# nomadkaraoke/python-audio-separator

Measured on AMD Instinct MI355X. Metric: audio-sec separated / wall-sec (RTF), UVR-MDX-NET 44.1kHz stereo, 1/2/4/8 GPU, higher is better.
Workload: dtype f32 (I/O and accumulators; matrix products on the 16-bit pipe from block-scaled two-part fp16 operands, 22-bit products -- see arithmetic; fp32-exact setting timed in arithmetic_ab)

## Files before the change

### python-audio-separator_amd/csrc/asx.hip

```cpp
#include <hip/hip_runtime.h>

#include <algorithm>
#include <atomic>
#include <cmath>
#include <cstdarg>
#include <cstdio>
#include <cstdlib>
#include <cstring>
#include <functional>
#include <map>
#include <string>
#include <mutex>
#include <vector>

#include "../../include/asx.h"
#include "knobs.h"
#include "resample_plan.h"
#include "flac_dec_plan.h"

static void grant_lds(const void *kernel, int bytes) {
  static std::mutex mu;
  static std::map<const void *, int> granted;
  std::lock_guard<std::mutex> lock(mu);
  int &g = granted[kernel];
// ... 43 lines not shown
  int (*norm)(int32_t);
  const char *refusal = nullptr;
  int shipped = 0;
} kOptions[] = {
    {"winograd", &asx_engine::winograd, &EngineKnobs::winograd, opt_nonneg,
     "asx_set_option: winograd = %d names a superseded kernel generation that only an experimental build carries "
     "(python build.py --experimental); this library has 0 (direct kernel) and 3 (the default)", 3},
    {"winograd_stationary", &asx_engine::winos, &EngineKnobs::winos, opt_nonneg,
     "asx_set_option: the weight-stationary Winograd kernel (measured slower) is in experimental builds only (python build.py --experimental)"},
    {"winograd_bf16x6", &asx_engine::wino6, &EngineKnobs::wino6, opt_nonneg},
    {"gemm_bf16x6", &asx_engine::gemm_bf16x6, &EngineKnobs::gemm_bf16x6, opt_onoff},
    {"gemm_f16x3", &asx_engine::gemm_f16x3, &EngineKnobs::gemm_f16x3, opt_onoff},
    {"conv_direct_f16x3", &asx_engine::conv3h, &EngineKnobs::conv3h, opt_nonneg},
    {"conv_fuse_input", &asx_engine::conv_fuse_input, &EngineKnobs::conv_fuse_input, opt_onoff},
    {"conv3h_partial_scratch", &asx_engine::conv3h_ps, &EngineKnobs::conv3h_ps, opt_onoff},
    {"conv_down_bf16x6", &asx_engine::down6, &EngineKnobs::down6, opt_onoff},
    {"conv_up_bf16x6", &asx_engine::up6, &EngineKnobs::up6, opt_onoff},
    {"gemm_pair_images", &asx_engine::pair_images, &EngineKnobs::pair_images, opt_onoff,
     "asx_set_option: gemm_pair_images = 1 needs an experimental build (python build.py --experimental): the pair-image reader measured no "
     "faster in the nets and is not in the default library"},
};

static const EngineOption *find_option(const char *fn, const char *key) {
  for (const EngineOption &o : kOptions)
    if (!strcmp(key, o.key)) return &o;
  set_err("%s: unknown option '%s'", fn, key);
  return nullptr;
}

extern "C" {
// ... 186 lines not shown
  e->d_tw3.release();
  e->d_hann3.release();
  e->seam3.release();
  e->d_zeros.release();
  free_conv(e->first);
  free_conv(e->final_);
  for (auto &b : e->enc) free_block(b);
  for (auto &b : e->dec) free_block(b);
  free_block(e->mid);
  for (auto &c : e->ds) free_conv(c);
  for (auto &c : e->us) free_conv(c);
  e->spec_in.release();
  e->spec_out.release();
  for (auto &r : e->R) r.release();
  e->c3h_ps.release();
  e->H.release();
  e->frames.release();
  e->chunk_out.release();
  e->d_starts.release();
  e->d_nact.release();
  e->d_peak.release();
  e->d_demixed.release();
  e->d_div.release();
  for (DevBuf *b : {&e->pool_wave, &e->pool_nsong, &e->pool_songs, &e->pool_div, &e->pool_peak}) b->release();
  for (auto &sk : e->skip) sk.release();
  if (e->v3) v3_destroy(e->v3);
  if (e->rof) rof_destroy(e->rof);
  hd_drop_clones(e);
  if (e->ht) ht_destroy(e->ht);
  if (e->hd) hd_destroy(e->hd);
// ... 251 lines not shown
  hipStream_t s = reinterpret_cast<hipStream_t>(stream);
  HIPCHK(hipSetDevice(e->device));
  asx_plan p;
  CHK(asx_plan_query(e, N, flags, &p));
  REQUIRE(k0 >= 0 && k1 <= p.n_chunks && k0 <= k1, "chunk range [%d,%d) outside [0,%d)", k0, k1, p.n_chunks);
  const bool match = (flags & ASX_FLAG_MATCH_MIX) != 0;
  const bool need_net = !match;
  if (need_net && !e->net_ready) {
    set_err("asx_demix: net weights not committed");
    return ASX_ERR_STATE;
  }
  const int nk = k1 - k0;
  if (nk == 0) return ASX_OK;
  const int per = even_batches(nk, pick_batch(e));
  CHK(ensure_workspace(e, per, need_net));
  const bool win = windowed_mode(e, flags);
  CHK(e->d_starts.ensure((size_t)nk * 8));
  CHK(e->d_nact.ensure((size_t)nk * 8));
  hipLaunchKernelGGL(chunk_table_kernel, dim3((unsigned)((nk + 255) / 256)), dim3(256), 0, s, k0, nk, p.step, p.chunk_size,
                     p.padded_len, win ? 1 : 0, reinterpret_cast<int64_t *>(e->d_starts.p), reinterpret_cast<int64_t *>(e->d_nact.p));
  HIPCHK(hipGetLastError());
  const int T = e->cfg.segment_size;
  const int64_t C = p.chunk_size;
  const size_t spec_elems = (size_t)4 * T * e->cfg.dim_f;
  for (int b0 = 0; b0 < nk; b0 += per) {
    const int B = std::min(per, nk - b0);
    const int64_t *ds = reinterpret_cast<const int64_t *>(e->d_starts.p) + b0;
    const int64_t *dn = reinterpret_cast<const int64_t *>(e->d_nact.p) + b0;
    CHK(stft_launch(e, mix_dev, ds, N, B, C, T, e->spec_in.f(), 1, 3, 1.0f, s));
    const float *spec_final = e->spec_in.f();
// ... 87 lines not shown
  }
  const int nk = (int)total;
  const asx_plan &p0 = plans[0];
  const int64_t C = p0.chunk_size;
  const int T = e->cfg.segment_size;
  const bool win = windowed_mode(e, flags);
  const double *hann = (e->fft3 && e->d_hann3.p) ? reinterpret_cast<const double *>(e->d_hann3.p) : nullptr;
  const int maxB = pick_batch(e);
  const int nbatch = (nk + maxB - 1) / maxB;
  const int per = (nk + nbatch - 1) / nbatch;
  std::map<int64_t, int64_t> div_off;
  int64_t div_floats = 0;
  for (int i = 0; i < n; ++i)
    if (div_off.emplace(Ns[i], div_floats).second) div_floats += (Ns[i] + 3) / 4 * 4;
  CHK(ensure_workspace(e, per, need_net));
  CHK(e->d_starts.ensure((size_t)nk * 8));
  CHK(e->d_nact.ensure((size_t)nk * 8));
  CHK(e->pool_wave.ensure((size_t)nk * 8));
  CHK(e->pool_nsong.ensure((size_t)nk * 8));
  CHK(e->pool_songs.ensure((size_t)n * sizeof(PoolSong)));
  CHK(e->pool_div.ensure((size_t)div_floats * 4));
  CHK(e->chunk_out.ensure((size_t)nk * 2 * C * 4));
  if (e->fft3) CHK(e->seam3.ensure((size_t)per * 2 * std::max(1, T / knobs().fft3_g) * 2 * 5 * f3::HOP * 4));
  float *chunks = e->chunk_out.f();
  const bool geom4 = knobs().finalize4 && C % 4 == 0 && p0.step % 4 == 0 && p0.trim % 4 == 0;
  int64_t blk = 0;
  for (int g0 = 0; g0 < n; g0 += POOL_GROUP) {
    PoolGroup g{};
    g.n_songs = std::min(POOL_GROUP, n - g0);
    g.song0 = g0;
// ... 641 lines not shown
  } else {
    set_err("asx_op_conv: unknown op '%s'", op);
    return ASX_ERR_INVALID;
  }
  ConvLayer L;
  DevBuf dx, dy, dskip;
  BufGuard g{{&dx, &dy, &dskip, &L.w, &L.b, &L.wu, &L.wu2, &L.wu3, &L.wus, &L.wu6, &L.wu6h, &L.w3h, &L.wd6, &L.wup6}};
  CHK(conv_setup(L, kind, cin, cout, relu ? 1 : 0));
  CHK(conv_pack(L, w_host, b_host, e->winograd));
  CHK(to_dev(dx, x_host, (size_t)B * cin * t * f));
  const size_t ny = (size_t)B * cout * to * fo;
  CHK(dy.ensure(ny * 4));
  HIPCHK(hipMemset(dy.p, 0xff, ny * 4));
  if (kind == CK_UP) CHK(to_dev(dskip, aux_host, ny));
  CHK(e->c3h_ps.ensure(conv3h_ps_need(L, B, t, f)));
  CHK(conv_launch(e, L, dx.f(), dskip.f(), dy.f(), B, t, f, nullptr));
  CHK(to_host(y_host, dy, ny));
  return ASX_OK;
}

int asx_op_tdf(asx_engine *e, const float *x_host, int32_t B, int32_t c, int32_t t, int32_t k, const float *w_host,
               const float *bias_host, int32_t n, const float *scale_host, const float *shift_host,
               const float *res_host, float *y_host) {
  REQUIRE(e && x_host && w_host && scale_host && shift_host && y_host && B > 0 && c > 0 && t > 0 && k > 0 && n > 0,
          "asx_op_tdf: bad argument");
  HIPCHK(hipSetDevice(e->device));
  TdfLayer L;
  DevBuf dx, dy, dres;
  BufGuard g{{&dx, &dy, &dres, &L.w, &L.bias, &L.scale, &L.shift}};
  CHK(tdf_pack(L, n, k, c, w_host, bias_host, scale_host, shift_host));
// ... 572 lines not shown
    if (br.rof)
      hipLaunchKernelGGL(roformer_finalize_pool_kernel, dim3((unsigned)blocks, br.rows * 2), dim3(256), 0, s, table, n, br.S, C, pp.step,
                         e->rof->d_window.f());
    else
      hipLaunchKernelGGL(mdxc_finalize_pool_kernel, dim3((unsigned)blocks, br.rows * 2), dim3(256), 0, s, table, n, br.S, C, pp.step, pp.front,
                         (float)pp.overlap);
  });
}

static int mdxc_pool_demix(asx_engine *e, const char *fn, bool rof, const asx_mdxc_song *songs, const MdxcPoolPlan &pp, void *stream) {
  hipStream_t s = reinterpret_cast<hipStream_t>(stream);
  HIPCHK(hipSetDevice(e->device));
  const MdxcBranch br = mdxc_branch(e, rof);
  const int nk = pp.total(), per = mdxc_pool_per_pass(nk, e->cfg.max_batch);
  CHK(rof ? rof_ensure_workspace(e, per) : v3_ensure_workspace(e, per));
  CHK(br.chunk_out.ensure((size_t)nk * br.chunk_floats(pp) * 4));
  int64_t blk = 0;
  CHK(mdxc_pool_tables(e, fn, br, songs, pp, br.chunk_out.f(), s, &blk));
  CHK(mdxc_pool_chunks(e, br, pp, 0, nk, br.chunk_out.f(), s));
  return mdxc_pool_fold(e, br, songs, pp, blk, s);
}

static int mdxc_pool_plan(const char *fn, asx_engine *e, bool rof, const asx_mdxc_song *songs, int32_t n_songs, int64_t geom, MdxcPoolPlan &pp) {
  REQUIRE(e && n_songs >= 0 && (songs || n_songs == 0), "%s: null argument", fn);
  std::vector<int64_t> Ns((size_t)n_songs);
  for (int i = 0; i < n_songs; ++i) {
    REQUIRE(songs[i].mix_dev && songs[i].out_dev, "%s: null pointer in song %d", fn, i);
    REQUIRE(songs[i].n_samples >= 1, "%s: song %d: n_samples must be >= 1", fn, i);
    Ns[i] = songs[i].n_samples;
  }
// ... 746 lines not shown
```

### python-audio-separator_amd/csrc/engine_core.h

```cpp
#pragma once

static thread_local char g_err[512] = "";
static void set_err(const char *fmt, ...) {
  va_list ap;
  va_start(ap, fmt);
  vsnprintf(g_err, sizeof(g_err), fmt, ap);
  va_end(ap);
}
#define HIPCHK(x)                                                                       \
  do {                                                                                  \
    hipError_t e_ = (x);                                                                \
    if (e_ != hipSuccess) {                                                             \
      set_err("%s:%d %s -> %s", __FILE__, __LINE__, #x, hipGetErrorString(e_));         \
      return ASX_ERR_HIP;                                                               \
    }                                                                                   \
  } while (0)
#define CHK(x)                    \
  do {                            \
    int r_ = (x);                 \
    if (r_ != ASX_OK) return r_;  \
  } while (0)
#define REQUIRE(cond, ...)        \
  do {                            \
    if (!(cond)) {                \
// ... 92 lines not shown
struct Block {
  std::vector<ConvLayer> tfc;
  TdfLayer tdf0, tdf1;
  int c = 0, t = 0, f = 0;
};

struct ProfRec {
  int cls;
  int nprod;
  hipEvent_t a, b;
  double flops, bytes;
};

struct RsTable {
  ResamplePlan plan;
  DevBuf tab;
};

struct V3Net;
struct RofNet;
struct HtNet;
struct HdNet;
struct VrNet;
struct EnsCtx;

struct W3Entry {
  const float *w;
  int N, K, cin;
  int kind;
  void *img;
// ... 30 lines not shown
  DevBuf d_tw3, seam3;
  bool fft3 = false;
  bool fft3p = false;
  DevBuf d_zeros;
  bool net_begun = false, net_ready = false;
  asx_net_config net{};
  std::map<std::string, std::vector<float>> host_tensors;
  ConvLayer first, final_;
  std::vector<Block> enc, dec;
  Block mid;
  std::vector<ConvLayer> ds, us;
  int ws_batch = 0;
  DevBuf spec_in, spec_out, R[3], H, HE, frames, chunk_out, d_starts, d_nact, d_peak, d_demixed;
  DevBuf pool_wave, pool_nsong, pool_songs, pool_div, pool_peak;
  DevBuf c3h_ps;
  DevBuf gn_part;
  DevBuf d_div;
  DivKey div_key;
  DevBuf sinc_tab;
  DevBuf flac_cycles;
  long long flac_block_cycles = 0, flac_crc16_cycles = 0;
  DevBuf flac_frames, flac_off;
  DevBuf flacdec_list, flacdec_slots, flacdec_accept;
  std::vector<flacdec::Accept> flacdec_accept_host;
  int64_t flacdec_n_samples = -1, flacdec_n_frames = 0;
  int32_t flacdec_channels = 0, flacdec_bps = 0, flacdec_max_bs = 0;
  size_t flacdec_slot_off = 0;
  std::vector<RsTable *> rs_tabs;
  std::mutex rs_mu;
  hipEvent_t div_ev = nullptr;
  hipStream_t div_stream = nullptr;
  std::vector<DevBuf> skip;
  int winograd = 3;
  int winos = 0;
  int gemm_bf16x6 = 1;
  int gemm_f16x3 = 1;
  int wino6 = 144;
  int conv3h = 144;
  int conv3h_ps = 1;
  int conv_fuse_input = 1;
  int down6 = 1;
  int up6 = 1;
  int pair_images = 0;
  std::vector<W3Entry> w3;
  std::mutex w3_mu;
  bool prof = false;
  int prof_nprod = 0;
  std::vector<ProfRec> recs;
};

static int pick_batch(const asx_engine *e) { return e->cfg.max_batch > 0 ? e->cfg.max_batch : 64; }

#include "batching.h"

// ... 74 lines not shown
```

### python-audio-separator_amd/csrc/engine_mdx.h

```cpp
#pragma once

template <class CFG>
static void launch_conv_t(const ConvArgs &a, int nblk, hipStream_t s) {
  grant_lds(&conv_mfma_kernel<CFG>, CFG::LDS_BYTES);
  hipLaunchKernelGGL(conv_mfma_kernel<CFG>, dim3(nblk), dim3(256), CFG::LDS_BYTES, s, a);
}

static int conv_tile_h(int kind) { return kind == CK_UP ? 4 : 8; }

static int pick_nrep_conv(int cout) {
  const int ct = (cout + 15) / 16;
  int best = 1, best_pad = 1 << 30;
  for (int n = 3; n >= 1; --n) {
    const int pad = ((ct + n - 1) / n) * n - ct;
    if (pad < best_pad) {
      best_pad = pad;
      best = n;
    }
  }
  return best;
}
static int pick_nrep_up(int cout) {
  const int ct = (cout + 15) / 16;
  if (knobs().up_nrep == 4 && (4 * ct) % 4 == 0) return 4;
// ... 207 lines not shown

static bool conv3h_takes(const asx_engine *e, const ConvLayer &L, bool dma, const float *res, int act, int T, int F, int64_t y_bstride, const float *y) {
#ifdef ASX_EXPERIMENTAL_KERNELS
  if (e->winos == 1 && L.wus.p != nullptr) return false;
#endif
  return L.kind == CK_3X3 && e->winograd == 3 && e->gemm_bf16x6 > 0 && e->gemm_f16x3 > 0 && e->conv3h > 0 && L.cin <= e->conv3h && L.w3h.p != nullptr && dma &&
         res == nullptr && (act == ACT_RELU || act == ACT_NONE) && F % 32 == 0 && (int64_t)Conv3hCfg::C * T * F < ((int64_t)1 << 29) &&
         y_bstride % 4 == 0 && (reinterpret_cast<uintptr_t>(y) & 15) == 0;
}

static size_t conv3h_ps_need(const ConvLayer &L, int B, int T, int F) {
  if (L.kind != CK_3X3 || L.w3h.p == nullptr || L.cin <= Conv3hCfg::C || F % 32 != 0 || B <= 0 || T <= 0) return 0;
  return (size_t)Conv3hCfg::ps_bytes(B, (T + 3) / 4, F / 32);
}

static int conv_launch(asx_engine *e, const ConvLayer &L, const float *x, const float *skip, float *y, int B, int T,
                       int F, hipStream_t s, const ConvView &v = ConvView()) {
  ConvArgs a{};
  a.x = x;
  a.wp = L.w.f();
  a.bias = L.b.f();
  a.skip = skip;
  a.res = v.res;
  a.zeros = e->d_zeros.f();
  a.y = y;
  a.B = B;
  a.Cin = L.cin;
  a.Cout = L.cout;
  a.T = T;
  a.F = F;
// ... 70 lines not shown
        case 1: return k12 ? gos(&conv_winos_kernel<12, 1>, WinoSCfg<12>::LDS_BYTES) : gos(&conv_winos_kernel<24, 1>, WinoSCfg<24>::LDS_BYTES);
        case 2: return k12 ? gos(&conv_winos_kernel<12, 2>, WinoSCfg<12>::LDS_BYTES) : gos(&conv_winos_kernel<24, 2>, WinoSCfg<24>::LDS_BYTES);
        case 4: return k12 ? gos(&conv_winos_kernel<12, 4>, WinoSCfg<12>::LDS_BYTES) : gos(&conv_winos_kernel<24, 4>, WinoSCfg<24>::LDS_BYTES);
        case 5: return k12 ? gos(&conv_winos_kernel<12, 5>, WinoSCfg<12>::LDS_BYTES) : gos(&conv_winos_kernel<24, 5>, WinoSCfg<24>::LDS_BYTES);
        case 13: return k12 ? gos(&conv_winos_kernel<12, 13>, WinoSCfg<12>::LDS_BYTES) : gos(&conv_winos_kernel<24, 13>, WinoSCfg<24>::LDS_BYTES);
        default: break;
      }
    }
    if (ragged) return k12 ? gos(&conv_winos_kernel<12, 0, true>, WinoSCfg<12>::LDS_BYTES) : gos(&conv_winos_kernel<24, 0, true>, WinoSCfg<24>::LDS_BYTES);
    return k12 ? gos(&conv_winos_kernel<12, 0, false>, WinoSCfg<12>::LDS_BYTES) : gos(&conv_winos_kernel<24, 0, false>, WinoSCfg<24>::LDS_BYTES);
  }
#endif
  if (conv3h_takes(e, L, dma, v.res, a.act, T, F, a.y_bstride, y)) {
    const int nb = L.cin / Conv3hCfg::C;
    const int tilesT = (T + 3) / 4, tilesF = F / 32;
    int bw = 32;
    double best = 1e30;
    for (int cand : {32, 16, 8}) {
      if ((tilesT * cand) % 32 != 0) continue;
      const int tps = tilesT * cand / 32;
      const int bands = (tilesF + cand - 1) / cand, items = B * bands;
      const double cost = (double)(bands * cand) / tilesF * (tps + 1.0) / tps * (double)((items + 7) / 8) / (items / 8.0);
      if (cost < best - 1e-9) {
        best = cost;
        bw = cand;
      }
    }
    if (best > 1e29) bw = 32;
    grant_lds(&conv3h_kernel<0, false>, Conv3hCfg::LDS_BYTES);
    grant_lds(&conv3h_kernel<0, true>, Conv3hCfg::LDS_BYTES);
    grant_lds(&conv3h_kernel<0, false, true>, Conv3hCfg::LDS_BYTES);
    grant_lds(&conv3h_kernel<0, false, false, 1>, Conv3hCfg::LDS_BYTES);
    grant_lds(&conv3h_kernel<0, false, false, 2>, Conv3hCfg::LDS_BYTES);
    grant_lds(&conv3h_kernel<0, false, false, 3>, Conv3hCfg::LDS_BYTES);
    const int64_t plane = (int64_t)T * F;
    const bool ps = e->conv3h_ps > 0 && nb > 1;
    const int64_t ps_item = Conv3hCfg::ps_item_bytes(tilesT, tilesF);
    REQUIRE(!ps || (ps_item < ((int64_t)1 << 32) && e->c3h_ps.p != nullptr && e->c3h_ps.bytes >= conv3h_ps_need(L, B, T, F)),
            "conv3h_kernel: the partial-sum scratch is not sized for %d x %d x %d (the workspace set-up sizes it)", B, T, F);
    Conv3hArgs walk{};
    walk.B = B;
    walk.T = T;
    walk.F = F;
    walk.x_bstride = a.x_bstride;
    walk.y_bstride = a.y_bstride;
    walk.tilesT = tilesT;
    walk.tilesF = tilesF;
    walk.bw = bw;
    walk.tps = (tilesT * bw) % 32 == 0 ? tilesT * bw / 32 : tilesT;
    walk.ps = ps ? e->c3h_ps.p : nullptr;
    walk.ps_bstride = ps_item;
    return timed(e, cls, flops, bytes, s, [&]() {
      e->prof_nprod = 3;
      for (int ob = 0; ob < nb; ++ob)
        for (int ib = 0; ib < nb; ++ib) {
          Conv3hArgs ca = walk;
          ca.x = x + (int64_t)ib * Conv3hCfg::C * plane;
          ca.y = y + (int64_t)ob * Conv3hCfg::C * plane;
          ca.prev = ib > 0 && !ps ? ca.y : nullptr;
          ca.wimg = reinterpret_cast<const u32x4 *>(reinterpret_cast<const uint32_t *>(L.w3h.p) + (size_t)(ob * nb + ib) * Conv3hCfg::IMG_U32);
          ca.bias = ib == 0 ? L.b.f() + ob * Conv3hCfg::C : nullptr;
          ca.act = ib == nb - 1 ? a.act : ACT_NONE;
          if (v.fin) {
            ca.xin = v.fin_x;
// ... 796 lines not shown
    for (int r = 0; r < 3; ++r)
      if (e->R[r].f() != cur) {
        out = e->R[r].f();
        break;
      }
    CHK(conv_launch(e, e->us[i], cur, gn ? nullptr : e->skip[n - 1 - i].f(), out, B, blk.t / 2, blk.f / 2, s));
    if (gn)
      CHK(gn_launch(e, out, B, e->us[i].cout, (int64_t)blk.t * blk.f, e->us[i].gn_w, e->us[i].gn_b, nullptr, e->skip[n - 1 - i].f(), out, s));
    cur = out;
    CHK(block_forward(e, blk, cur, nullptr, B, s));
  }
  CHK(conv_launch(e, e->final_, cur, nullptr, spec_out, B, T, F, s));
  return ASX_OK;
}

static int ensure_workspace(asx_engine *e, int Bchunks, bool need_net) {
  const int T = e->cfg.segment_size, Fq = e->cfg.dim_f;
  const int mult = (need_net && e->cfg.enable_denoise) ? 2 : 1;
  const size_t Bn = (size_t)Bchunks * mult;
  CHK(e->spec_in.ensure(Bn * 4 * T * Fq * 4));
  CHK(e->frames.ensure((size_t)Bchunks * 2 * T * e->cfg.n_fft * 4));
  if (need_net) {
    CHK(e->spec_out.ensure(Bn * 4 * T * Fq * 4));
    const size_t lvl0 = Bn * e->net.g * T * Fq * 4;
    for (int i = 0; i < 3; ++i) CHK(e->R[i].ensure(lvl0));
    CHK(e->H.ensure(Bn * e->net.g * T * (Fq / std::max(1, e->net.bn)) * 4 + 256));
    CHK(e->HE.ensure(Bn * e->net.g * T * (size_t)((Fq / std::max(1, e->net.bn) + 127) / 128) * 4 + 256));
    if (e->net.norm == 1) CHK(e->gn_part.ensure(Bn * (size_t)e->net.g * (e->net.num_blocks / 2 + 1) * 16));
    const int n = e->net.num_blocks / 2;
    e->skip.resize(n);
    for (int i = 0; i < n; ++i) {
      const size_t c = (size_t)e->net.g * (i + 1), t = T >> i, f = Fq >> i;
      CHK(e->skip[i].ensure(Bn * c * t * f * 4));
    }
    size_t ps = 0;
    auto ps_block = [&](const Block &blk) {
      for (const ConvLayer &L : blk.tfc) ps = std::max(ps, conv3h_ps_need(L, (int)Bn, blk.t, blk.f));
    };
    for (const Block &blk : e->enc) ps_block(blk);
    ps_block(e->mid);
    for (const Block &blk : e->dec) ps_block(blk);
    CHK(e->c3h_ps.ensure(ps));
  }
  e->ws_batch = std::max(e->ws_batch, Bchunks);
  return ASX_OK;
}
```

### python-audio-separator_amd/csrc/engine_v3.h

```cpp
#pragma once
#include "v3_norm.h"

struct V3Norm {
  DevBuf g, b;
  int c = 0;
};

struct V3Block {
  int in_c = 0, c = 0, f = 0;
  V3Norm n_tfc1, n_tdf0, n_tdf1, n_tfc2;
  ConvLayer tfc1, tfc2, shortcut;
  TdfLayer tdf0, tdf1;
};

struct V3Net {
  asx_v3_config cfg{};
  float act_alpha = 1.f;
  bool begun = false, ready = false;
  ConvLayer first, final0, final1;
  std::vector<std::vector<V3Block>> enc, dec;
  std::vector<V3Block> mid;
  std::vector<ConvLayer> ds, us;
  std::vector<V3Norm> ds_n, us_n;
  int ws_batch = 0;
// ... 160 lines not shown
    CHK(tdf_launch(e, b.tdf0, n.A.f(), nullptr, n.H.f(), M, T, s, 0));
    const int fb = b.tdf0.n;
    CHK(v3_norm_act(e, b.n_tdf1, V3View{n.H.f(), (int64_t)b.c * T * fb}, b.c, (int64_t)T * fb, B, n.HA.f(), s));
    CHK(tdf_launch(e, b.tdf1, n.HA.f(), n.X1.f(), n.X2.f(), M, T, s, 0));
    CHK(v3_norm_act(e, b.n_tfc2, V3View{n.X2.f(), (int64_t)b.c * P}, b.c, P, B, n.A.f(), s));
    ConvView vo;
    vo.res = n.S.f();
    V3View out = last ? dest : V3View{n.XB.f(), (int64_t)b.c * P};
    vo.y_bstride = out.bstride;
    CHK(conv_launch(e, b.tfc2, n.A.f(), nullptr, out.p, B, T, F, s, vo));
    x = out;
  }
  return ASX_OK;
}

static int v3_ensure_workspace(asx_engine *e, int B) {
  V3Net &n = *e->v3;
  if (B <= n.ws_batch) return ASX_OK;
  const asx_v3_config &cf = n.cfg;
  const int T = e->cfg.segment_size, k = cf.num_subbands, Fs = e->cfg.dim_f / k;
  const int dim_c = k * cf.num_channels * 2;
  const int64_t P0 = (int64_t)T * Fs;
  const int c0 = cf.num_channels_model;
  const size_t big = (size_t)B * 2 * c0 * P0 * 4;
  CHK(n.cat0.ensure((size_t)B * (dim_c + c0) * P0 * 4));
  CHK(n.firstout.ensure((size_t)B * c0 * P0 * 4));
  CHK(n.A.ensure(big));
  CHK(n.S.ensure(big / 2));
  CHK(n.X1.ensure(big / 2));
  CHK(n.X2.ensure(big / 2));
  CHK(n.XB.ensure(big / 2));
  CHK(n.CUR.ensure(big / 2));
// ... 186 lines not shown
```

### python-audio-separator_amd/csrc/kernels_conv3h.h

```cpp
#pragma once
#include <cstring>
#include <vector>

#include "kernels_gemm3.h"

namespace asx {

struct Conv3hArgs {
  const float *x;
  float *y;
  const u32x4 *wimg;
  const float *bias;
  int B, T, F;
  int64_t x_bstride, y_bstride;
  int act;
  int tilesT, tilesF;
  int bw, tps;
  const float *prev;
  long long *dbg;
  const float *xin;
  const float *w1;
  int64_t xin_bstride;
  void *ps;
  int64_t ps_bstride;
};

struct Conv3hCfg {
  static constexpr int C = 48, CG8 = C / 8;
  static constexpr int TH = 4, TW = 32, IW = TW + 2;
  static constexpr int PSTR = C * 2;
  static constexpr int ROWB = IW * PSTR;
  static constexpr int RING = 12;
  static constexpr int PART = RING * ROWB;
  static constexpr int KGY = 3 * CG8;
  static constexpr int SPK = (KGY + 3) / 4;
  static constexpr int NST = (3 * KGY + 3) / 4;
  static constexpr int WKY = (KGY / 4) * 3 * 2 * 1024 + 3 * 2 * 512;
  static constexpr int WBYTES = 3 * WKY;
  static constexpr int W_OFF = 0, X_OFF = WBYTES, TAB_OFF = X_OFF + 2 * PART;
  static constexpr int LDS_BYTES = TAB_OFF + 64;
  static constexpr size_t IMG_U32 = WBYTES / 4 + 48;
  static constexpr int EUP = 8;

  static constexpr int PS_STORE = 1024, PS_WAVE = 6 * PS_STORE, PS_TILE = 4 * PS_WAVE;
  static constexpr int64_t ps_item_bytes(int tilesT, int tilesF) { return (int64_t)tilesF * tilesT * PS_TILE; }
  static constexpr int64_t ps_bytes(int B, int tilesT, int tilesF) { return (int64_t)B * ps_item_bytes(tilesT, tilesF); }
  static constexpr unsigned ps_wave_off(int tilesT, int strip, int jt, int r) { return (unsigned)((strip * tilesT + jt) * 4 + r) * (unsigned)PS_WAVE; }
  static constexpr int64_t ps_off(int tilesT, int tilesF, int b, int strip, int jt, int r, int k, int lane) {
    return (int64_t)b * ps_item_bytes(tilesT, tilesF) + ps_wave_off(tilesT, strip, jt, r) + k * PS_STORE + lane * 16;
  }

  enum { FULL = 0, MERGED = 1, PADDED = 2 };
  struct Stage {
    int kind, ky, kyb, sg;
    int rfrom, rto;
  };
  static constexpr int NPROG = 2;
// ... 104 lines not shown
            hh[e] = conv3h_f16_rne(us);
            ll[e] = conv3h_f16_rne(us - conv3h_f16_f(hh[e]));
          }
          const size_t pstep = half ? 512 : 1024;
          const size_t fb = (size_t)ky * CFG::WKY + (half ? (size_t)(CFG::SPK - 1) * 6144 + (size_t)(n * 2) * 512 : (size_t)sg * 6144 + (size_t)(n * 2) * 1024);
          uint32_t *dh = &img[(fb + (size_t)lane * 16) / 4], *dl = &img[(fb + pstep + (size_t)lane * 16) / 4];
          for (int e = 0; e < 4; ++e) {
            dh[e] = (uint32_t)hh[2 * e] | ((uint32_t)hh[2 * e + 1] << 16);
            dl[e] = (uint32_t)ll[2 * e] | ((uint32_t)ll[2 * e + 1] << 16);
          }
        }
    }
}

struct Conv3hWalk {
  int item, j, b, strip;
};
__device__ __forceinline__ void conv3h_walk_item(const Conv3hArgs &a, int wg, Conv3hWalk &w) {
  const int nbands = (a.tilesF + a.bw - 1) / a.bw;
  w.b = w.item / nbands;
  w.strip = (w.item - w.b * nbands) * a.bw + (wg >> 3) % a.bw;
}
__device__ __forceinline__ int conv3h_row0(const Conv3hArgs &a, int wg) { return ((wg >> 3) / a.bw) * a.tps * 4; }
__device__ __forceinline__ int conv3h_nblocks(const Conv3hArgs &a, int wg) {
  const int items = a.B * ((a.tilesF + a.bw - 1) / a.bw), x = wg & 7;
  return x < items ? ((items - x + 7) >> 3) * (a.tps + 1) : 0;
}
__device__ __forceinline__ void conv3h_walk_init(const Conv3hArgs &a, int wg, Conv3hWalk &w) {
  w.item = wg & 7;
  w.j = -1;
  conv3h_walk_item(a, wg, w);
}
__device__ __forceinline__ void conv3h_walk_next(const Conv3hArgs &a, int wg, Conv3hWalk &w) {
  if (++w.j == a.tps) {
    w.j = -1;
    w.item += 8;
    conv3h_walk_item(a, wg, w);
  }
}

__device__ __forceinline__ void conv3h_split_pair(float x0, float x1, float s, unsigned &h, unsigned &l) {
  unsigned hh = 0, ll = 0;
  asm("v_fma_mixlo_f16 %0, %1, %2, 0 op_sel_hi:[0,0,0]" : "+v"(hh) : "v"(x0), "v"(s));
  asm("v_fma_mixhi_f16 %0, %1, %2, 0 op_sel_hi:[0,0,0]" : "+v"(hh) : "v"(x1), "v"(s));
  asm("v_fma_mixlo_f16 %0, %1, %2, -%3 op_sel:[0,0,0] op_sel_hi:[0,0,1]" : "+v"(ll) : "v"(x0), "v"(s), "v"(hh));
  asm("v_fma_mixhi_f16 %0, %1, %2, -%3 op_sel:[0,0,1] op_sel_hi:[0,0,1]" : "+v"(ll) : "v"(x1), "v"(s), "v"(hh));
  h = hh;
  l = ll;
}

template <int BM>
__device__ __forceinline__ float ror8m(float keep, float from) {
// ... 17 lines not shown
  extern __shared__ float lds_f[];
  char *lds = reinterpret_cast<char *>(lds_f);
  const int tid = threadIdx.x;
  const int lane = tid & 63;
  const int wave = __builtin_amdgcn_readfirstlane(tid >> 6);
  const int wg = blockIdx.x;
  float *maxtab = reinterpret_cast<float *>(lds + CFG::TAB_OFF);
  int *exps = reinterpret_cast<int *>(lds + CFG::TAB_OFF + 32);

  {
    const u32x4 *src = a.wimg;
    u32x4 *dst = reinterpret_cast<u32x4 *>(lds + CFG::W_OFF);
    for (int i = tid; i < CFG::WBYTES / 16; i += 512) dst[i] = src[i];
  }
  const int64_t TF = (int64_t)a.T * a.F;
  const int NB = conv3h_nblocks(a, wg);
  const int row0 = conv3h_row0(a, wg);
  const unsigned plane_bytes = (unsigned)(CFG::C * TF * 4);

  if (wave >= 4) {
    const int ptid = tid - 256, pw = wave - 4;
    int row, cig, q;
    if (ptid < 160) {
      q = (ptid & 1) + 2 * ((ptid >> 3) % 5);
      cig = (ptid >> 1) & 3;
      row = ptid / 40;
    } else {
      const int u = ptid - 160;
      q = (u & 1) + 2 * ((u >> 3) % 5);
      cig = 4 + ((u >> 1) & 1);
      row = ((u >> 2) & 1) + 2 * (u / 40);
    }
// ... 11 lines not shown
        const f32x4 wv = *reinterpret_cast<const f32x4 *>(a.w1 + (cig * 8 + c) * 4);
        fr.w1[c][0] = wv.x;
        fr.w1[c][1] = wv.y;
        fr.w1[c][2] = wv.z;
        fr.w1[c][3] = wv.w;
        fr.b1[c] = a.w1[CFG::C * 4 + cig * 8 + c];
      }
    }

    Conv3hWalk wk;
    conv3h_walk_init(a, wg, wk);
    int nf = 0;
    auto fetch = [&](auto setc) {
      constexpr int S = decltype(setc)::value;
      const int tb = nf < NB ? wk.b : 0, f0 = wk.strip * 32;
      const int t1 = nf < NB ? row0 + wk.j * 4 + 1 : -(1 << 20);
      ++nf;
      conv3h_walk_next(a, wg, wk);
      __amdgpu_buffer_rsrc_t rs = FIN ? __builtin_amdgcn_make_buffer_rsrc(const_cast<float *>(a.xin + (int64_t)tb * a.xin_bstride), 0, in_bytes, 0x00020000)
                                      : __builtin_amdgcn_make_buffer_rsrc(const_cast<float *>(a.x + (int64_t)tb * a.x_bstride), 0, plane_bytes, 0x00020000);
      const int org = t1 * a.F + (f0 - 4);
      const bool ok = item_ok && (unsigned)(t1 + row) < (unsigned)a.T && (unsigned)(f0 - 4 + 4 * q) < (unsigned)a.F;
      const unsigned vo = ok ? (unsigned)(goff + org) * 4u : 0xfffffff0u;
      if constexpr (FIN) {
        fr.ok[S] = ok;
#pragma unroll
        for (int j = 0; j < 4; ++j) fr.rin[S][j] = __builtin_bit_cast(f32x4, __builtin_amdgcn_raw_buffer_load_b128(rs, (int)vo, (int)(j * TF * 4), 0));
      } else {
#pragma unroll
        for (int j = 0; j < 8; ++j) {
          if constexpr ((ABL & 2) != 0) raw[S][j] = (f32x4){0.25f, 0.5f, 0.75f, 1.f};
// ... 19 lines not shown
      for (int j = 0; j < 8; ++j) {
        m = __builtin_fmaxf(__builtin_fmaxf(m, __builtin_fabsf(raw[S][j].x)), __builtin_fabsf(raw[S][j].y));
        m = __builtin_fmaxf(__builtin_fmaxf(m, __builtin_fabsf(raw[S][j].z)), __builtin_fabsf(raw[S][j].w));
      }
      m = wave_max64(m);
      if (!(m <= 3.4028234663852886e38f)) {
        m = 0.f;
#pragma unroll
        for (int j = 0; j < 8; ++j) {
          m = fmaxf(m, fmaxf(fmaxf(finite_or_zero(raw[S][j].x), finite_or_zero(raw[S][j].y)), fmaxf(finite_or_zero(raw[S][j].z), finite_or_zero(raw[S][j].w))));
        }
        m = wave_max64(m);
      }
      if (lane == 0) maxtab[slot * 4 + pw] = m;
    };
    int e_prev = 0, js = -1;
    auto split_store = [&](auto setc, int par, int slot3) {
      constexpr int S = decltype(setc)::value % NSET;
      const f32x4 mv = *reinterpret_cast<const f32x4 *>(maxtab + par * 4);
      const float m = fmaxf(fmaxf(mv.x, mv.y), fmaxf(mv.z, mv.w));
      int need = f16_scale_exp(m) - 1;
      need = need < 100 ? need : 100;
      int e = e_prev;
      if (js < 0 || need < e_prev) e = need;
      else if (need > e_prev + CFG::EUP) e = need < e_prev + 40 ? need : e_prev + 40;
      e_prev = e;
      if (++js == a.tps) js = -1;
      if (ptid == 0) exps[slot3] = e;
      const float sc = __builtin_ldexpf(1.0f, e);
      char *dst = lds + CFG::X_OFF + slot3 * 4 * CFG::ROWB + loff;
      if constexpr ((ABL & 8) != 0) return;
#pragma unroll
      for (int i = 0; i < 4; ++i) {
        unsigned hh[4], ll[4];
#pragma unroll
        for (int c2 = 0; c2 < 4; ++c2) conv3h_split_pair(raw[S][2 * c2][i], raw[S][2 * c2 + 1][i], sc, hh[c2], ll[c2]);
        const bool wok = item_ok && (i == 3 ? q <= 8 : (i == 0 ? q >= 1 : (q >= 1 && q <= 8)));
        if (wok) {
          *reinterpret_cast<u32x4 *>(dst + i * CFG::PSTR) = (u32x4){hh[0], hh[1], hh[2], hh[3]};
          *reinterpret_cast<u32x4 *>(dst + CFG::PART + i * CFG::PSTR) = (u32x4){ll[0], ll[1], ll[2], ll[3]};
        }
      }
// ... 141 lines not shown
      flush_one(IntC<0>{});
      flush_one(IntC<1>{});
      flush_one(IntC<2>{});
      flush_one(IntC<3>{});
      flush_one(IntC<4>{});
      flush_one(IntC<5>{});
      pend_rs = __builtin_amdgcn_make_buffer_rsrc(a.y, 0, 0, 0x00020000);
    };

    __syncthreads();
    __syncthreads();
    Conv3hWalk wk;
    conv3h_walk_init(a, wg, wk);
    int s3 = 0;
    for (int s = 0; s < NB; ++s) {
      const int tb = wk.b, j = wk.j, wk_strip = wk.strip, f0 = wk_strip * 32;
      conv3h_walk_next(a, wg, wk);
      if constexpr ((ABL & 32) != 0) {
        if (wg == 0 && wave == 0 && s < 64) {
          const long long t = __builtin_amdgcn_s_memtime();
          if (lane == 0) a.dbg[s * 8 + 4] = t;
        }
      }
      if (j >= 0) {
        const int tt = row0 + j * 4 + wave;
        const bool cur_ok = tt < a.T && f0 < a.F;
        const int cur_vo = (((li & 7) * a.T + tt) * a.F + f0 + ((li >> 3) * 4 + g) * 4) * 4;
        const int cur_ps = (int)CFG::ps_wave_off(a.tilesT, wk_strip, (row0 >> 2) + j, wave);
        const int sp = s3 == 0 ? 2 : s3 - 1;
        const int e_cur = __builtin_amdgcn_readfirstlane(exps[s3]), e_old = __builtin_amdgcn_readfirstlane(exps[sp]);
        int rowoff[3], eky[3];
#pragma unroll
        for (int ky = 0; ky < 3; ++ky) {
          const int u = wave + ky;
          rowoff[ky] = (u < 2 ? sp * 4 + 2 + u : s3 * 4 + u - 2) * CFG::ROWB;
          eky[ky] = u < 2 ? e_old : e_cur;
        }
        const int xm = (pad_lane ? rowoff[MST.kyb] : rowoff[MST.ky]) + vl[CFG::SPK - 1];
        f32x4 acc[2][3];
#pragma unroll
        for (int p = 0; p < 2; ++p)
#pragma unroll
          for (int c = 0; c < 3; ++c) acc[p][c] = (f32x4){0.f, 0.f, 0.f, 0.f};
// ... 133 lines not shown
```

### python-audio-separator_amd/csrc/knobs.h

```cpp
#pragma once

#include <algorithm>
#include <climits>
#include <cstdint>
#include <cstdlib>

#ifndef ASX_TDF2_DEFAULT
#define ASX_TDF2_DEFAULT 1
#endif

constexpr int HD_MAX_GROUPS = 6;

namespace knob {
inline bool set(const char *name) { return getenv(name) != nullptr; }
inline int num(const char *name, int def) { return set(name) ? atoi(getenv(name)) : def; }
inline int64_t num64(const char *name, int64_t def) { return set(name) ? atoll(getenv(name)) : def; }
inline double real(const char *name, double def) { return set(name) ? atof(getenv(name)) : def; }
inline bool on_unless_0(const char *name) { return !(set(name) && atoi(getenv(name)) == 0); }
inline bool off_unless_nonzero(const char *name) { return set(name) && atoi(getenv(name)) != 0; }
inline int clamped(const char *name, int def, int lo, int hi = INT_MAX) { return set(name) ? std::max(lo, std::min(hi, atoi(getenv(name)))) : def; }
}

struct Knobs {
  int poison = knob::num("ASX_POISON", -1);
// ... 67 lines not shown
#ifdef ASX_EXPERIMENTAL_KERNELS
  int winograd = knob::clamped("ASX_WINOGRAD", 3, 0);
  int winos = knob::clamped("ASX_WINOS", 0, 0);
  int pair_images = knob::num("ASX_PAIR_IMAGES", 0);
#else
  int winograd = knob::num("ASX_WINOGRAD", 3) <= 0 ? 0 : 3;
  int winos = 0;
  int pair_images = 0;
#endif
  int gemm_bf16x6 = knob::num("ASX_GEMM_BF16X6", 1);
  int gemm_f16x3 = knob::num("ASX_GEMM_F16X3", 1);
  int wino6 = knob::clamped("ASX_WINO6", 144, 0);
  int conv3h = knob::clamped("ASX_CONV3H", 144, 0);
  int conv_fuse_input = 1;
  int conv3h_ps = 1;
  int down6 = knob::num("ASX_DOWN6", 1);
  int up6 = knob::num("ASX_UP6", 1);
  bool fft3 = knob::on_unless_0("ASX_FFT3");
  bool fft3p = knob::on_unless_0("ASX_FFT3P");
};
```

Before: 1665.

## Drive conv3h workgroup walk from host-planned balanced unit tables

```diff
diff --git a/python-audio-separator_amd/csrc/asx.hip b/python-audio-separator_amd/csrc/asx.hip
--- a/python-audio-separator_amd/csrc/asx.hip
+++ b/python-audio-separator_amd/csrc/asx.hip
@@ -81,6 +81,7 @@
     {"conv_direct_f16x3", &asx_engine::conv3h, &EngineKnobs::conv3h, opt_nonneg},
     {"conv_fuse_input", &asx_engine::conv_fuse_input, &EngineKnobs::conv_fuse_input, opt_onoff},
     {"conv3h_partial_scratch", &asx_engine::conv3h_ps, &EngineKnobs::conv3h_ps, opt_onoff},
+    {"conv3h_walk", &asx_engine::conv3h_walk, &EngineKnobs::conv3h_walk, opt_onoff},
     {"conv_down_bf16x6", &asx_engine::down6, &EngineKnobs::down6, opt_onoff},
     {"conv_up_bf16x6", &asx_engine::up6, &EngineKnobs::up6, opt_onoff},
     {"gemm_pair_images", &asx_engine::pair_images, &EngineKnobs::pair_images, opt_onoff,
@@ -297,6 +298,11 @@
   e->spec_out.release();
   for (auto &r : e->R) r.release();
   e->c3h_ps.release();
+  for (Conv3hWalkTab *t : e->c3h_walks) {
+    t->tab.release();
+    delete t;
+  }
+  e->c3h_walks.clear();
   e->H.release();
   e->frames.release();
   e->chunk_out.release();
@@ -578,6 +584,7 @@
   if (nk == 0) return ASX_OK;
   const int per = even_batches(nk, pick_batch(e));
   CHK(ensure_workspace(e, per, need_net));
+  if (need_net && nk % per) CHK(net_walks_ensure(e, (nk % per) * (e->cfg.enable_denoise ? 2 : 1)));
   const bool win = windowed_mode(e, flags);
   CHK(e->d_starts.ensure((size_t)nk * 8));
   CHK(e->d_nact.ensure((size_t)nk * 8));
@@ -695,6 +702,7 @@
   for (int i = 0; i < n; ++i)
     if (div_off.emplace(Ns[i], div_floats).second) div_floats += (Ns[i] + 3) / 4 * 4;
   CHK(ensure_workspace(e, per, need_net));
+  if (need_net && nk % per) CHK(net_walks_ensure(e, (nk % per) * (e->cfg.enable_denoise ? 2 : 1)));
   CHK(e->d_starts.ensure((size_t)nk * 8));
   CHK(e->d_nact.ensure((size_t)nk * 8));
   CHK(e->pool_wave.ensure((size_t)nk * 8));
@@ -1366,6 +1374,7 @@
   HIPCHK(hipMemset(dy.p, 0xff, ny * 4));
   if (kind == CK_UP) CHK(to_dev(dskip, aux_host, ny));
   CHK(e->c3h_ps.ensure(conv3h_ps_need(L, B, t, f)));
+  CHK(conv3h_walk_ensure(e, L, B, t, f));
   CHK(conv_launch(e, L, dx.f(), dskip.f(), dy.f(), B, t, f, nullptr));
   CHK(to_host(y_host, dy, ny));
   return ASX_OK;
@@ -1968,6 +1977,7 @@
   const MdxcBranch br = mdxc_branch(e, rof);
   const int nk = pp.total(), per = mdxc_pool_per_pass(nk, e->cfg.max_batch);
   CHK(rof ? rof_ensure_workspace(e, per) : v3_ensure_workspace(e, per));
+  if (!rof && nk % per) CHK(v3_walks_ensure(e, nk % per));
   CHK(br.chunk_out.ensure((size_t)nk * br.chunk_floats(pp) * 4));
   int64_t blk = 0;
   CHK(mdxc_pool_tables(e, fn, br, songs, pp, br.chunk_out.f(), s, &blk));
diff --git a/python-audio-separator_amd/csrc/conv3h_walk_plan.h b/python-audio-separator_amd/csrc/conv3h_walk_plan.h
--- /dev/null
+++ b/python-audio-separator_amd/csrc/conv3h_walk_plan.h
@@ -0,0 +1,127 @@
+#pragma once
+#include <algorithm>
+#include <cstdint>
+#include <vector>
+
+struct Conv3hUnit {
+  int32_t b, band, t0, tiles;
+};
+
+struct Conv3hWalkPlan {
+  int bw = 32, tps = 0;
+  int ngroups = 8;
+  std::vector<std::vector<Conv3hUnit>> units;
+  int steps(int g) const {
+    int n = 0;
+    for (const Conv3hUnit &u : units[(size_t)g]) n += u.tiles + 1;
+    return n;
+  }
+  int longest() const {
+    int n = 0;
+    for (int g = 0; g < ngroups; ++g) n = std::max(n, steps(g));
+    return n;
+  }
+  int max_units() const {
+    size_t n = 0;
+    for (const auto &l : units) n = std::max(n, l.size());
+    return (int)n;
+  }
+};
+
+static inline int conv3h_walk_bw0(int B, int tilesT, int tilesF) {
+  int bw = 32;
+  double best = 1e30;
+  for (int cand : {32, 16, 8}) {
+    if ((tilesT * cand) % 32 != 0) continue;
+    const int tps = tilesT * cand / 32;
+    const int bands = (tilesF + cand - 1) / cand, items = B * bands;
+    const double cost = (double)(bands * cand) / tilesF * (tps + 1.0) / tps * (double)((items + 7) / 8) / (items / 8.0);
+    if (cost < best - 1e-9) {
+      best = cost;
+      bw = cand;
+    }
+  }
+  return best > 1e29 ? 32 : bw;
+}
+
+static inline Conv3hWalkPlan conv3h_walk_arith(int B, int tilesT, int tilesF, int bw) {
+  Conv3hWalkPlan p;
+  p.bw = (tilesT * bw) % 32 == 0 ? bw : 32;
+  p.tps = tilesT * p.bw / 32;
+  const int segs = 32 / p.bw, nbands = (tilesF + p.bw - 1) / p.bw, items = B * nbands;
+  p.ngroups = 8 * segs;
+  p.units.assign((size_t)p.ngroups, {});
+  for (int x = 0; x < 8; ++x)
+    for (int seg = 0; seg < segs; ++seg)
+      for (int item = x; item < items; item += 8)
+        p.units[(size_t)(x * segs + seg)].push_back({item / nbands, item % nbands, seg * p.tps, p.tps});
+  return p;
+}
+static inline Conv3hWalkPlan conv3h_walk_plan0(int B, int tilesT, int tilesF) { return conv3h_walk_arith(B, tilesT, tilesF, conv3h_walk_bw0(B, tilesT, tilesF)); }
+
+static inline Conv3hWalkPlan conv3h_walk_balanced(int B, int tilesT, int tilesF, int gran, int bw) {
+  Conv3hWalkPlan p;
+  p.bw = bw;
+  p.tps = 0;
+  p.ngroups = 256 / bw;
+  p.units.assign((size_t)p.ngroups, {});
+  const int G = p.ngroups, nbands = (tilesF + bw - 1) / bw, items = B * nbands;
+  const int rounds = items / G, left = items - rounds * G;
+  for (int r = 0; r < rounds; ++r)
+    for (int g = 0; g < G; ++g) {
+      const int item = r * G + g;
+      p.units[(size_t)g].push_back({item / nbands, item % nbands, 0, tilesT});
+    }
+  if (left > 0) {
+    const int64_t tT = ((int64_t)(tilesT + gran - 1) / gran) * gran, total = (int64_t)left * tT;
+    int64_t share = (total + G - 1) / G;
+    share = (share + gran - 1) / gran * gran;
+    for (int g = 0; g < G; ++g) {
+      int64_t lo = (int64_t)g * share;
+      const int64_t hi = std::min(total, lo + share);
+      while (lo < hi) {
+        const int64_t i = lo / tT, t0 = lo - i * tT, t1 = std::min<int64_t>(tT, t0 + (hi - lo));
+        const int item = rounds * G + (int)i;
+        if (t0 < tilesT) p.units[(size_t)g].push_back({item / nbands, item % nbands, (int)t0, (int)std::min<int64_t>(t1, tilesT) - (int)t0});
+        lo += t1 - t0;
+      }
+    }
+  }
+  return p;
+}
+
+static inline Conv3hWalkPlan conv3h_walk_plan(int B, int tilesT, int tilesF, int gran, int mode) {
+  Conv3hWalkPlan best = conv3h_walk_plan0(B, tilesT, tilesF);
+  if (mode == 0) return best;
+  if (gran < 1) gran = 1;
+  int nbest = best.tps % gran == 0 || best.tps == tilesT ? best.longest() : INT32_MAX;
+  for (int bw : {32, 16, 8}) {
+    Conv3hWalkPlan c = conv3h_walk_balanced(B, tilesT, tilesF, gran, bw);
+    const int n = c.longest();
+    if (n < nbest) {
+      nbest = n;
+      best = std::move(c);
+    }
+  }
+  return best;
+}
+
+static inline int conv3h_walk_table(const Conv3hWalkPlan &p, std::vector<int32_t> &tab) {
+  const int stride = p.max_units() + 2;
+  tab.assign((size_t)p.ngroups * stride * 4, 0);
+  for (int g = 0; g < p.ngroups; ++g) {
+    int32_t *row = &tab[(size_t)g * stride * 4];
+    const auto &l = p.units[(size_t)g];
+    row[0] = p.steps(g);
+    row[1] = (int32_t)l.size();
+    for (size_t u = 0; u <= l.size(); ++u) {
+      const Conv3hUnit un = u < l.size() ? l[u] : Conv3hUnit{0, 0, 0, 1 << 30};
+      int32_t *e = row + 4 * (1 + u);
+      e[0] = un.b;
+      e[1] = un.band;
+      e[2] = un.t0;
+      e[3] = un.tiles;
+    }
+  }
+  return stride;
+}
diff --git a/python-audio-separator_amd/csrc/engine_core.h b/python-audio-separator_amd/csrc/engine_core.h
--- a/python-audio-separator_amd/csrc/engine_core.h
+++ b/python-audio-separator_amd/csrc/engine_core.h
@@ -130,6 +130,12 @@
 
 struct RsTable {
   ResamplePlan plan;
+  DevBuf tab;
+};
+
+struct Conv3hWalkTab {
+  int B, tilesT, tilesF, mode;
+  int bw, stride;
   DevBuf tab;
 };
 
@@ -190,6 +196,7 @@
   DevBuf spec_in, spec_out, R[3], H, HE, frames, chunk_out, d_starts, d_nact, d_peak, d_demixed;
   DevBuf pool_wave, pool_nsong, pool_songs, pool_div, pool_peak;
   DevBuf c3h_ps;
+  std::vector<Conv3hWalkTab *> c3h_walks;
   DevBuf gn_part;
   DevBuf d_div;
   DivKey div_key;
@@ -214,6 +221,7 @@
   int wino6 = 144;
   int conv3h = 144;
   int conv3h_ps = 1;
+  int conv3h_walk = 1;
   int conv_fuse_input = 1;
   int down6 = 1;
   int up6 = 1;
diff --git a/python-audio-separator_amd/csrc/engine_mdx.h b/python-audio-separator_amd/csrc/engine_mdx.h
--- a/python-audio-separator_amd/csrc/engine_mdx.h
+++ b/python-audio-separator_amd/csrc/engine_mdx.h
@@ -245,6 +245,34 @@
   return (size_t)Conv3hCfg::ps_bytes(B, (T + 3) / 4, F / 32);
 }
 
+static const Conv3hWalkTab *conv3h_walk_find(const asx_engine *e, int B, int tilesT, int tilesF, int mode) {
+  for (const Conv3hWalkTab *t : e->c3h_walks)
+    if (t->B == B && t->tilesT == tilesT && t->tilesF == tilesF && t->mode == mode) return t;
+  return nullptr;
+}
+static int conv3h_walk_ensure(asx_engine *e, const ConvLayer &L, int B, int T, int F) {
+  if (L.kind != CK_3X3 || L.w3h.p == nullptr || F % 32 != 0 || B <= 0 || T <= 0) return ASX_OK;
+  const int tilesT = (T + 3) / 4, tilesF = F / 32;
+  for (int mode = 0; mode < 2; ++mode) {
+    if (conv3h_walk_find(e, B, tilesT, tilesF, mode)) continue;
+    const Conv3hWalkPlan plan = conv3h_walk_plan(B, tilesT, tilesF, 1, mode);
+    std::vector<int32_t> tab;
+    Conv3hWalkTab *t = new Conv3hWalkTab{B, tilesT, tilesF, mode, plan.bw, conv3h_walk_table(plan, tab), DevBuf()};
+    int rc = t->tab.ensure(tab.size() * 4);
+    if (rc == ASX_OK && hipMemcpy(t->tab.p, tab.data(), tab.size() * 4, hipMemcpyHostToDevice) != hipSuccess) {
+      set_err("conv3h_walk_ensure: the upload of a walk table failed");
+      rc = ASX_ERR_HIP;
+    }
+    if (rc != ASX_OK) {
+      t->tab.release();
+      delete t;
+      return rc;
+    }
+    e->c3h_walks.push_back(t);
+  }
+  return ASX_OK;
+}
+
 static int conv_launch(asx_engine *e, const ConvLayer &L, const float *x, const float *skip, float *y, int B, int T,
                        int F, hipStream_t s, const ConvView &v = ConvView()) {
   ConvArgs a{};
@@ -345,19 +373,8 @@
   if (conv3h_takes(e, L, dma, v.res, a.act, T, F, a.y_bstride, y)) {
     const int nb = L.cin / Conv3hCfg::C;
     const int tilesT = (T + 3) / 4, tilesF = F / 32;
-    int bw = 32;
-    double best = 1e30;
-    for (int cand : {32, 16, 8}) {
-      if ((tilesT * cand) % 32 != 0) continue;
-      const int tps = tilesT * cand / 32;
-      const int bands = (tilesF + cand - 1) / cand, items = B * bands;
-      const double cost = (double)(bands * cand) / tilesF * (tps + 1.0) / tps * (double)((items + 7) / 8) / (items / 8.0);
-      if (cost < best - 1e-9) {
-        best = cost;
-        bw = cand;
-      }
-    }
-    if (best > 1e29) bw = 32;
+    const Conv3hWalkTab *wt = conv3h_walk_find(e, B, tilesT, tilesF, e->conv3h_walk > 0 ? 1 : 0);
+    REQUIRE(wt != nullptr, "conv3h_kernel: no walk table for %d x %d x %d (the workspace set-up plans them)", B, T, F);
     grant_lds(&conv3h_kernel<0, false>, Conv3hCfg::LDS_BYTES);
     grant_lds(&conv3h_kernel<0, true>, Conv3hCfg::LDS_BYTES);
     grant_lds(&conv3h_kernel<0, false, true>, Conv3hCfg::LDS_BYTES);
@@ -377,8 +394,9 @@
     walk.y_bstride = a.y_bstride;
     walk.tilesT = tilesT;
     walk.tilesF = tilesF;
-    walk.bw = bw;
-    walk.tps = (tilesT * bw) % 32 == 0 ? tilesT * bw / 32 : tilesT;
+    walk.bw = wt->bw;
+    walk.walk = reinterpret_cast<const u32x4 *>(wt->tab.p);
+    walk.walk_stride = wt->stride;
     walk.ps = ps ? e->c3h_ps.p : nullptr;
     walk.ps_bstride = ps_item;
     return timed(e, cls, flops, bytes, s, [&]() {
@@ -1205,6 +1223,17 @@
   return ASX_OK;
 }
 
+static int net_walks_ensure(asx_engine *e, int Bn) {
+  auto walks = [&](const Block &blk) -> int {
+    for (const ConvLayer &L : blk.tfc) CHK(conv3h_walk_ensure(e, L, Bn, blk.t, blk.f));
+    return ASX_OK;
+  };
+  for (const Block &blk : e->enc) CHK(walks(blk));
+  CHK(walks(e->mid));
+  for (const Block &blk : e->dec) CHK(walks(blk));
+  return ASX_OK;
+}
+
 static int ensure_workspace(asx_engine *e, int Bchunks, bool need_net) {
   const int T = e->cfg.segment_size, Fq = e->cfg.dim_f;
   const int mult = (need_net && e->cfg.enable_denoise) ? 2 : 1;
@@ -1232,6 +1261,7 @@
     ps_block(e->mid);
     for (const Block &blk : e->dec) ps_block(blk);
     CHK(e->c3h_ps.ensure(ps));
+    CHK(net_walks_ensure(e, (int)Bn));
   }
   e->ws_batch = std::max(e->ws_batch, Bchunks);
   return ASX_OK;
diff --git a/python-audio-separator_amd/csrc/engine_v3.h b/python-audio-separator_amd/csrc/engine_v3.h
--- a/python-audio-separator_amd/csrc/engine_v3.h
+++ b/python-audio-separator_amd/csrc/engine_v3.h
@@ -198,8 +198,27 @@
   return ASX_OK;
 }
 
+static int v3_walks_ensure(asx_engine *e, int B) {
+  V3Net &n = *e->v3;
+  const asx_v3_config &cf = n.cfg;
+  auto walks = [&](const std::vector<V3Block> &bs, int t, int f) -> int {
+    for (const V3Block &b : bs) {
+      CHK(conv3h_walk_ensure(e, b.tfc1, B, t, f));
+      CHK(conv3h_walk_ensure(e, b.tfc2, B, t, f));
+    }
+    return ASX_OK;
+  };
+  int t = e->cfg.segment_size, f = e->cfg.dim_f / cf.num_subbands;
+  for (int i = 0; i < cf.num_scales; ++i, t /= 2, f /= 2) {
+    CHK(walks(n.enc[i], t, f));
+    CHK(walks(n.dec[cf.num_scales - 1 - i], t, f));
+  }
+  return walks(n.mid, t, f);
+}
+
 static int v3_ensure_workspace(asx_engine *e, int B) {
   V3Net &n = *e->v3;
+  CHK(v3_walks_ensure(e, B));
   if (B <= n.ws_batch) return ASX_OK;
   const asx_v3_config &cf = n.cfg;
   const int T = e->cfg.segment_size, k = cf.num_subbands, Fs = e->cfg.dim_f / k;
diff --git a/python-audio-separator_amd/csrc/kernels_conv3h.h b/python-audio-separator_amd/csrc/kernels_conv3h.h
--- a/python-audio-separator_amd/csrc/kernels_conv3h.h
+++ b/python-audio-separator_amd/csrc/kernels_conv3h.h
@@ -2,6 +2,7 @@
 #include <cstring>
 #include <vector>
 
+#include "conv3h_walk_plan.h"
 #include "kernels_gemm3.h"
 
 namespace asx {
@@ -15,7 +16,9 @@
   int64_t x_bstride, y_bstride;
   int act;
   int tilesT, tilesF;
-  int bw, tps;
+  int bw;
+  const u32x4 *walk;
+  int walk_stride;
   const float *prev;
   long long *dbg;
   const float *xin;
@@ -41,6 +44,7 @@
   static constexpr int LDS_BYTES = TAB_OFF + 64;
   static constexpr size_t IMG_U32 = WBYTES / 4 + 48;
   static constexpr int EUP = 8;
+  static constexpr int EQ = 8;
 
   static constexpr int PS_STORE = 1024, PS_WAVE = 6 * PS_STORE, PS_TILE = 4 * PS_WAVE;
   static constexpr int64_t ps_item_bytes(int tilesT, int tilesF) { return (int64_t)tilesF * tilesT * PS_TILE; }
@@ -175,28 +179,31 @@
 }
 
 struct Conv3hWalk {
-  int item, j, b, strip;
+  int u, j, b, strip, t0, tiles;
 };
-__device__ __forceinline__ void conv3h_walk_item(const Conv3hArgs &a, int wg, Conv3hWalk &w) {
-  const int nbands = (a.tilesF + a.bw - 1) / a.bw;
-  w.b = w.item / nbands;
-  w.strip = (w.item - w.b * nbands) * a.bw + (wg >> 3) % a.bw;
-}
-__device__ __forceinline__ int conv3h_row0(const Conv3hArgs &a, int wg) { return ((wg >> 3) / a.bw) * a.tps * 4; }
-__device__ __forceinline__ int conv3h_nblocks(const Conv3hArgs &a, int wg) {
-  const int items = a.B * ((a.tilesF + a.bw - 1) / a.bw), x = wg & 7;
-  return x < items ? ((items - x + 7) >> 3) * (a.tps + 1) : 0;
-}
+__device__ __forceinline__ void conv3h_walk_unit(const Conv3hArgs &a, int wg, Conv3hWalk &w) {
+  const u32x4 un = a.walk[w.u];
+  w.b = __builtin_amdgcn_readfirstlane((int)un.x);
+  w.strip = __builtin_amdgcn_readfirstlane((int)un.y) * a.bw + ((wg >> 3) & (a.bw - 1));
+  w.t0 = __builtin_amdgcn_readfirstlane((int)un.z);
+  w.tiles = __builtin_amdgcn_readfirstlane((int)un.w);
+}
+__device__ __forceinline__ int conv3h_walk_row(const Conv3hArgs &a, int wg) {
+  const int sh = __builtin_ctz((unsigned)a.bw);
+  return ((wg & 7) * (32 >> sh) + ((wg >> 3) >> sh)) * a.walk_stride;
+}
+__device__ __forceinline__ int conv3h_row0(const Conv3hWalk &w) { return w.t0 * 4; }
+__device__ __forceinline__ int conv3h_nblocks(const Conv3hArgs &a, int wg) { return (int)a.walk[conv3h_walk_row(a, wg)].x; }
 __device__ __forceinline__ void conv3h_walk_init(const Conv3hArgs &a, int wg, Conv3hWalk &w) {
-  w.item = wg & 7;
+  w.u = conv3h_walk_row(a, wg) + 1;
   w.j = -1;
-  conv3h_walk_item(a, wg, w);
+  conv3h_walk_unit(a, wg, w);
 }
 __device__ __forceinline__ void conv3h_walk_next(const Conv3hArgs &a, int wg, Conv3hWalk &w) {
-  if (++w.j == a.tps) {
+  if (++w.j == w.tiles) {
     w.j = -1;
-    w.item += 8;
-    conv3h_walk_item(a, wg, w);
+    ++w.u;
+    conv3h_walk_unit(a, wg, w);
   }
 }
 
@@ -244,8 +251,7 @@
     for (int i = tid; i < CFG::WBYTES / 16; i += 512) dst[i] = src[i];
   }
   const int64_t TF = (int64_t)a.T * a.F;
-  const int NB = conv3h_nblocks(a, wg);
-  const int row0 = conv3h_row0(a, wg);
+  const int NB = __builtin_amdgcn_readfirstlane(conv3h_nblocks(a, wg));
   const unsigned plane_bytes = (unsigned)(CFG::C * TF * 4);
 
   if (wave >= 4) {
@@ -287,7 +293,7 @@
     auto fetch = [&](auto setc) {
       constexpr int S = decltype(setc)::value;
       const int tb = nf < NB ? wk.b : 0, f0 = wk.strip * 32;
-      const int t1 = nf < NB ? row0 + wk.j * 4 + 1 : -(1 << 20);
+      const int t1 = nf < NB ? conv3h_row0(wk) + wk.j * 4 + 1 : -(1 << 20);
       ++nf;
       conv3h_walk_next(a, wg, wk);
       __amdgpu_buffer_rsrc_t rs = FIN ? __builtin_amdgcn_make_buffer_rsrc(const_cast<float *>(a.xin + (int64_t)tb * a.xin_bstride), 0, in_bytes, 0x00020000)
@@ -337,18 +343,15 @@
       }
       if (lane == 0) maxtab[slot * 4 + pw] = m;
     };
-    int e_prev = 0, js = -1;
+    int e_prev = 0;
     auto split_store = [&](auto setc, int par, int slot3) {
       constexpr int S = decltype(setc)::value % NSET;
       const f32x4 mv = *reinterpret_cast<const f32x4 *>(maxtab + par * 4);
       const float m = fmaxf(fmaxf(mv.x, mv.y), fmaxf(mv.z, mv.w));
       int need = f16_scale_exp(m) - 1;
       need = need < 100 ? need : 100;
-      int e = e_prev;
-      if (js < 0 || need < e_prev) e = need;
-      else if (need > e_prev + CFG::EUP) e = need < e_prev + 40 ? need : e_prev + 40;
+      const int e = m > 0.f ? need & ~(CFG::EQ - 1) : e_prev;
       e_prev = e;
-      if (++js == a.tps) js = -1;
       if (ptid == 0) exps[slot3] = e;
       const float sc = __builtin_ldexpf(1.0f, e);
       char *dst = lds + CFG::X_OFF + slot3 * 4 * CFG::ROWB + loff;
@@ -520,7 +523,7 @@
     conv3h_walk_init(a, wg, wk);
     int s3 = 0;
     for (int s = 0; s < NB; ++s) {
-      const int tb = wk.b, j = wk.j, wk_strip = wk.strip, f0 = wk_strip * 32;
+      const int tb = wk.b, j = wk.j, wk_strip = wk.strip, wk_t0 = wk.t0, f0 = wk_strip * 32;
       conv3h_walk_next(a, wg, wk);
       if constexpr ((ABL & 32) != 0) {
         if (wg == 0 && wave == 0 && s < 64) {
@@ -529,10 +532,10 @@
         }
       }
       if (j >= 0) {
-        const int tt = row0 + j * 4 + wave;
+        const int tt = (wk_t0 + j) * 4 + wave;
         const bool cur_ok = tt < a.T && f0 < a.F;
         const int cur_vo = (((li & 7) * a.T + tt) * a.F + f0 + ((li >> 3) * 4 + g) * 4) * 4;
-        const int cur_ps = (int)CFG::ps_wave_off(a.tilesT, wk_strip, (row0 >> 2) + j, wave);
+        const int cur_ps = (int)CFG::ps_wave_off(a.tilesT, wk_strip, wk_t0 + j, wave);
         const int sp = s3 == 0 ? 2 : s3 - 1;
         const int e_cur = __builtin_amdgcn_readfirstlane(exps[s3]), e_old = __builtin_amdgcn_readfirstlane(exps[sp]);
         int rowoff[3], eky[3];
diff --git a/python-audio-separator_amd/csrc/knobs.h b/python-audio-separator_amd/csrc/knobs.h
--- a/python-audio-separator_amd/csrc/knobs.h
+++ b/python-audio-separator_amd/csrc/knobs.h
@@ -105,6 +105,7 @@
   int conv3h = knob::clamped("ASX_CONV3H", 144, 0);
   int conv_fuse_input = 1;
   int conv3h_ps = 1;
+  int conv3h_walk = 1;
   int down6 = knob::num("ASX_DOWN6", 1);
   int up6 = knob::num("ASX_UP6", 1);
   bool fft3 = knob::on_unless_0("ASX_FFT3");
```

New measurement: 1683, median of 6. 1.1% higher.
